# wolearyc/ramannoodle

Hardware: NVIDIA B200
Metric: md_frames_per_s (higher is better)
Workload: dtype f64

## Files before the change

ramannoodle_b200/csrc/rn_device.cuh:

```cuda
#pragma once

#include "rn_common.cuh"

namespace rn {

struct Alpha0 {
    double v[9];
};

__device__ __forceinline__ double wrap_disp(double pos, double ref) {
    const double d = pos - ref;
    return d - ceil(d - 0.5);
}

__device__ __forceinline__ double wrap_disp_fast(double pos, double ref) {
    const double d = pos - ref;
    const unsigned mag = (unsigned)__double2hiint(d) & 0x7fffffffu;
    if (mag < 0x3fe00000u) return d;
    return d - ceil(d - 0.5);
}

__device__ __forceinline__ void dmma884(double& c0, double& c1, double a, double b) {
    asm("mma.sync.aligned.m8n8k4.row.col.f64.f64.f64.f64 {%0,%1}, {%2}, {%3}, {%0,%1};"
        : "+d"(c0), "+d"(c1)
        : "d"(a), "d"(b));
}

__device__ __forceinline__ uint32_t smem_u32(const void* p) { return (uint32_t)__cvta_generic_to_shared(p); }

__device__ __forceinline__ void cp_async_16(uint32_t dst, const void* src, int src_bytes) {
    asm volatile("cp.async.cg.shared.global [%0], [%1], 16, %2;" ::"r"(dst), "l"(src), "r"(src_bytes) : "memory");
}
__device__ __forceinline__ void cp_async_8(uint32_t dst, const void* src, int src_bytes) {
    asm volatile("cp.async.ca.shared.global [%0], [%1], 8, %2;" ::"r"(dst), "l"(src), "r"(src_bytes) : "memory");
}
__device__ __forceinline__ void cp_async_commit() { asm volatile("cp.async.commit_group;" ::: "memory"); }
template <int N>
__device__ __forceinline__ void cp_async_wait() {
    asm volatile("cp.async.wait_group %0;" ::"n"(N) : "memory");
}

__device__ __forceinline__ void mbar_init(uint32_t bar, uint32_t count) {
    asm volatile("mbarrier.init.shared::cta.b64 [%0], %1;" ::"r"(bar), "r"(count) : "memory");
}
__device__ __forceinline__ void mbar_arrive_expect_tx(uint32_t bar, uint32_t bytes) {
    asm volatile("mbarrier.arrive.expect_tx.shared::cta.b64 _, [%0], %1;" ::"r"(bar), "r"(bytes) : "memory");
}
__device__ __forceinline__ void mbar_wait(uint32_t bar, uint32_t parity) {
    asm volatile(
        "{\n"
        ".reg .pred p;\n"
        "WAIT_%=:\n"
        "mbarrier.try_wait.parity.shared::cta.b64 p, [%0], %1;\n"
        "@p bra DONE_%=;\n"
        "bra WAIT_%=;\n"
        "DONE_%=:\n"
        "}\n" ::"r"(bar),
        "r"(parity)
        : "memory");
}
__device__ __forceinline__ void tma_bulk_g2s(uint32_t dst, const void* src, uint32_t bytes, uint32_t bar) {
    asm volatile("cp.async.bulk.shared::cluster.global.mbarrier::complete_tx::bytes [%0], [%1], %2, [%3];" ::"r"(dst),
                 "l"(src), "r"(bytes), "r"(bar)
                 : "memory");
}

}
```

ramannoodle_b200/csrc/rn_fft.cuh:

```cuda
#pragma once

#include "rn_common.cuh"

namespace rn {
namespace fft {

constexpr int kLog2E = 12;
constexpr int kE = 1 << kLog2E;
constexpr int kNT = 256;
constexpr int kPerThread = kE / kNT;
constexpr size_t kTileSmemBytes = (size_t)kE * sizeof(double2);

enum { OUT_PLAIN = 0, OUT_POWER = 1, OUT_PEERS = 2 };

__device__ __forceinline__ double2 cmul(double2 a, double2 b) {
    return make_double2(a.x * b.x - a.y * b.y, a.x * b.y + a.y * b.x);
}
__device__ __forceinline__ double2 cadd(double2 a, double2 b) { return make_double2(a.x + b.x, a.y + b.y); }
__device__ __forceinline__ double2 csub(double2 a, double2 b) { return make_double2(a.x - b.x, a.y - b.y); }
__device__ __forceinline__ double2 conj(double2 a) { return make_double2(a.x, -a.y); }

template <int SGN>
__device__ __forceinline__ double2 mul_i(double2 a) {
    return SGN > 0 ? make_double2(-a.y, a.x) : make_double2(a.y, -a.x);
}

template <int RADIX, int SGN>
struct Dft;

template <int SGN>
struct Dft<2, SGN> {
    static __device__ __forceinline__ void run(double2* v) {
        const double2 a = v[0];
        v[0] = cadd(a, v[1]);
        v[1] = csub(a, v[1]);
    }
};

template <int SGN>
struct Dft<4, SGN> {
    static __device__ __forceinline__ void run(double2* v) {
        const double2 s02 = cadd(v[0], v[2]), d02 = csub(v[0], v[2]);
        const double2 s13 = cadd(v[1], v[3]), d13 = mul_i<SGN>(csub(v[1], v[3]));
        v[0] = cadd(s02, s13);
        v[1] = cadd(d02, d13);
        v[2] = csub(s02, s13);
        v[3] = csub(d02, d13);
    }
};

template <int SGN>
struct Dft<8, SGN> {
    static __device__ __forceinline__ void run(double2* v) {
        double2 e[4] = {v[0], v[2], v[4], v[6]};
        double2 o[4] = {v[1], v[3], v[5], v[7]};
        Dft<4, SGN>::run(e);
        Dft<4, SGN>::run(o);
        const double h = 0.70710678118654752440;
        const double2 o1 = make_double2(h * (o[1].x - SGN * o[1].y), h * (SGN * o[1].x + o[1].y));
        const double2 o2 = mul_i<SGN>(o[2]);
        const double2 o3 = make_double2(h * (-o[3].x - SGN * o[3].y), h * (SGN * o[3].x - o[3].y));
        v[0] = cadd(e[0], o[0]);
        v[4] = csub(e[0], o[0]);
        v[1] = cadd(e[1], o1);
        v[5] = csub(e[1], o1);
        v[2] = cadd(e[2], o2);
        v[6] = csub(e[2], o2);
        v[3] = cadd(e[3], o3);
        v[7] = csub(e[3], o3);
    }
};

template <int RADIX>
struct Log2;
template <>
struct Log2<2> {
    static constexpr int value = 1;
};
template <>
struct Log2<4> {
    static constexpr int value = 2;
};
template <>
struct Log2<8> {
    static constexpr int value = 3;
};

template <int RADIX>
__device__ __forceinline__ void apply_powers(double2* x, double2 w1) {
    x[1] = cmul(x[1], w1);
    if constexpr (RADIX >= 4) {
        const double2 w2 = cmul(w1, w1);
        const double2 w3 = cmul(w2, w1);
        x[2] = cmul(x[2], w2);
        x[3] = cmul(x[3], w3);
        if constexpr (RADIX == 8) {
            const double2 w4 = cmul(w2, w2);
            x[4] = cmul(x[4], w4);
            x[5] = cmul(x[5], cmul(w4, w1));
            x[6] = cmul(x[6], cmul(w3, w3));
            x[7] = cmul(x[7], cmul(w4, w3));
        }
    }
}

template <int RADIX>
__device__ __forceinline__ void apply_base_step(double2* x, double2 base, double2 step) {
    double2 w = base;
#pragma unroll
    for (int q = 0; q < RADIX; q++) {
        x[q] = cmul(x[q], w);
        if (q + 1 < RADIX) w = cmul(w, step);
    }
}

__device__ __forceinline__ int swz(int pos) { return pos ^ ((pos >> 3) & 7); }

struct Twiddles {
    const double2* hi;
    const double2* lo;
    const double2* sub;
    int split;
};

__device__ __forceinline__ double2 tw_global(const Twiddles& T, uint32_t m) {
    return cmul(__ldg(T.hi + (m >> T.split)), __ldg(T.lo + (m & ((1u << T.split) - 1u))));
}

struct PeerOut {
    double2* ptr[8];
    int log2w;
    int log2lh;
    int rank;
    int world;
    int64_t c;
};

__host__ __device__ __forceinline__ int64_t mirror_half_slots(int log2w) { return ((int64_t)1 << (log2w - 1)) + 64; }

__device__ __forceinline__ void mirror_arcs(int o, int64_t c, int log2lh, int log2w, int64_t* near_origin,
                                            int64_t* far_top) {
    const int64_t lh = (int64_t)1 << log2lh;
    const int64_t a0 = ((int64_t)o << log2w) + (c & 1);
    *near_origin = (((c + a0) >> 1) & (lh - 1)) & ~(int64_t)31;
    *far_top = (((2 * lh + c - a0) >> 1) & (lh - 1)) | 31;
}

__device__ __forceinline__ void mirror_owner(int64_t m1, int64_t c, int log2lh, int log2w, int world, int* owner,
                                             int64_t* slot) {
    const int64_t lh = (int64_t)1 << log2lh;
    int64_t u = 2 * m1 - c;
    if (u < 0) u += 2 * lh;
    const bool far_side = u > lh;
    const int64_t a = far_side ? 2 * lh - u : u;
    const int o = min((int)(a >> log2w), world - 1);
    int64_t near_origin, far_top;
    mirror_arcs(o, c, log2lh, log2w, &near_origin, &far_top);
    *owner = o;
    *slot = far_side ? mirror_half_slots(log2w) + ((far_top - m1) & (lh - 1)) : ((m1 - near_origin) & (lh - 1));
}

struct OutSpec {
    int mode;
    double* power;
    int64_t M;
    PeerOut peers;
};

__device__ __forceinline__ void store_out(const OutSpec& out, double2* plain, int seq, int64_t m, double2 v) {
    if (out.mode == OUT_PLAIN) {
        *plain = v;
    } else if (out.mode == OUT_POWER) {
        if (m < out.M) out.power[(int64_t)seq * out.M + m] = v.x * v.x + v.y * v.y;
    } else {
        int owner;
        int64_t slot;
        mirror_owner(m, out.peers.c, out.peers.log2lh, out.peers.log2w, out.peers.world, &owner, &slot);
        const int64_t stride = 2 * mirror_half_slots(out.peers.log2w);
        out.peers.ptr[owner][(int64_t)(seq * out.peers.world + out.peers.rank) * stride + slot] = v;
    }
}

template <int SGN, int RADIX, bool LEAN, class Rd, class Wr>
__device__ __forceinline__ void fft_stage(int log2sp, int log2b, const double2* __restrict__ wsub, Rd rd, Wr wr) {
    constexpr int NB = kPerThread / RADIX;
    constexpr int LR = Log2<RADIX>::value;
    const int sp = 1 << log2sp;
    const int log2ns = log2sp - log2b + LR;
    const bool has_tw = log2sp > log2b;
#pragma unroll(LEAN ? 1 : NB)
    for (int m = 0; m < NB; m++) {
        const int u = (int)threadIdx.x + m * kNT;
        const int lo = u & (sp - 1);
        const int pos0 = ((u >> log2sp) << (log2sp + LR)) + lo;
        double2 x[RADIX];
#pragma unroll
        for (int q = 0; q < RADIX; q++) x[q] = rd(pos0 + (q << log2sp), m * RADIX + q);
        double2 w1 = make_double2(1.0, 0.0);
        if (has_tw) {
            w1 = __ldg(wsub + ((lo >> log2b) << (kLog2E - log2ns)));
            if (SGN > 0) w1.y = -w1.y;
        }
        if (SGN > 0 && has_tw) apply_powers<RADIX>(x, w1);
        Dft<RADIX, SGN>::run(x);
        if (SGN < 0 && has_tw) apply_powers<RADIX>(x, w1);
#pragma unroll
        for (int q = 0; q < RADIX; q++) wr(pos0 + (q << log2sp), m * RADIX + q, x[q]);
    }
}

struct TileParams {
    double2* X;
    int64_t seq_stride;
    int tiles_per_seq;
    const double2* H;
    double2* Hout;
    int64_t limit;
    int seq_base;
    OutSpec out;
    Twiddles tw;
};

template <bool FWD_ONLY, bool LEAN>
__global__ void __launch_bounds__(kNT, LEAN ? 3 : 2) tile_kernel(const __grid_constant__ TileParams P) {
    extern __shared__ __align__(16) unsigned char fft_smem[];
    double2* S = reinterpret_cast<double2*>(fft_smem);
    const int seq = blockIdx.x / P.tiles_per_seq;
    const int tile = blockIdx.x - seq * P.tiles_per_seq;
    const int64_t tile_base = (int64_t)tile * kE;
    double2* base = P.X + (int64_t)seq * P.seq_stride + tile_base;
    const double2* wsub = P.tw.sub;

    auto rd_s = [&](int pos, int) { return S[swz(pos)]; };
    auto wr_s = [&](int pos, int, double2 v) { S[swz(pos)] = v; };
    auto rd_g = [&](int pos, int) {
        return (tile_base + pos < P.limit) ? base[pos] : make_double2(0.0, 0.0);
    };

    fft_stage<-1, 8, LEAN>(9, 0, wsub, rd_g, wr_s);
    __syncthreads();
    fft_stage<-1, 8, LEAN>(6, 0, wsub, rd_s, wr_s);
    __syncthreads();
    fft_stage<-1, 8, LEAN>(3, 0, wsub, rd_s, wr_s);
    __syncthreads();
#pragma unroll(LEAN ? 1 : kPerThread / 8)
    for (int m = 0; m < kPerThread / 8; m++) {
        const int pos0 = ((int)threadIdx.x + m * kNT) << 3;
        double2 h[8];
        const int hu = (int)threadIdx.x + m * kNT;
        if (!FWD_ONLY) {
#pragma unroll
            for (int q = 0; q < 8; q++) h[q] = __ldg(P.H + tile_base + (q << 9) + hu);
        }
        double2 x[8];
#pragma unroll
        for (int q = 0; q < 8; q++) x[q] = S[swz(pos0 + q)];
        Dft<8, -1>::run(x);
        if (FWD_ONLY) {
#pragma unroll
            for (int q = 0; q < 8; q++) P.Hout[tile_base + (q << 9) + hu] = x[q];
        } else {
#pragma unroll
            for (int q = 0; q < 8; q++) x[q] = cmul(x[q], h[q]);
            Dft<8, +1>::run(x);
#pragma unroll
            for (int q = 0; q < 8; q++) S[swz(pos0 + q)] = x[q];
        }
    }
    if (FWD_ONLY) return;
    __syncthreads();
    fft_stage<+1, 8, LEAN>(3, 0, wsub, rd_s, wr_s);
    __syncthreads();
    fft_stage<+1, 8, LEAN>(6, 0, wsub, rd_s, wr_s);
    __syncthreads();
    auto wr_g = [&](int pos, int, double2 v) { store_out(P.out, base + pos, P.seq_base + seq, tile_base + pos, v); };
    fft_stage<+1, 8, LEAN>(9, 0, wsub, rd_s, wr_g);
}

struct LevelParams {
    double2* X;
    int64_t seq_stride;
    int log2lsub;
    int log2r;
    int nsub;
    int tw_shift;
    int64_t limit;
    int seq_base;
    OutSpec out;
    Twiddles tw;
};

__device__ __forceinline__ int rev3(int x, int groups) {
    int r = 0;
    for (int i = 0; i < groups; i++) {
        r = (r << 3) | (x & 7);
        x >>= 3;
    }
    return r;
}

template <int SGN>
struct LevelCtx {
    const LevelParams& P;
    double2* S;
    double2* base;
    int64_t elem_base;
    int seq;
    int log2b, log2s;
    int a8;
    int j0;
};

template <int SGN, int RADIX, bool SMEM_SIDE, bool LEAN>
__device__ __forceinline__ void level_twiddle_stage(const LevelCtx<SGN>& C) {
    constexpr int NB = kPerThread / RADIX;
    constexpr int LR = Log2<RADIX>::value;
    const LevelParams& P = C.P;
    const int B = 1 << C.log2b;
    const int groups = (P.log2r - LR) / 3;
#pragma unroll(LEAN ? 1 : (RADIX == 8 ? NB : 2))
    for (int m = 0; m < NB; m++) {
        const int u = (int)threadIdx.x + m * kNT;
        const int col = u & (B - 1);
        const int rb = u >> C.log2b;
        const int pos0 = (rb << (C.log2b + LR)) + col;
        const uint32_t j = (uint32_t)(C.j0 + col);
        const uint32_t krest = (uint32_t)rev3(rb, groups);
        double2 wb = tw_global(P.tw, (krest * j) << P.tw_shift);
        double2 ws = tw_global(P.tw, (j << (P.log2r - LR)) << P.tw_shift);
        if (SGN > 0) {
            wb.y = -wb.y;
            ws.y = -ws.y;
        }
        double2 x[RADIX];
        if (SGN < 0) {
#pragma unroll
            for (int q = 0; q < RADIX; q++) {
                const int pos = pos0 + (q << C.log2b);
                if (SMEM_SIDE) {
                    x[q] = C.S[swz(pos)];
                } else {
                    const int64_t off = ((int64_t)(pos >> C.log2b) << C.log2s) + (pos & (B - 1));
                    x[q] = (C.elem_base + off < P.limit) ? C.base[off] : make_double2(0.0, 0.0);
                }
            }
            Dft<RADIX, SGN>::run(x);
            apply_base_step<RADIX>(x, wb, ws);
#pragma unroll
            for (int q = 0; q < RADIX; q++) {
                const int pos = pos0 + (q << C.log2b);
                C.base[((int64_t)(pos >> C.log2b) << C.log2s) + (pos & (B - 1))] = x[q];
            }
        } else {
#pragma unroll
            for (int q = 0; q < RADIX; q++) {
                const int pos = pos0 + (q << C.log2b);
                x[q] = C.base[((int64_t)(pos >> C.log2b) << C.log2s) + (pos & (B - 1))];
            }
            apply_base_step<RADIX>(x, wb, ws);
            Dft<RADIX, SGN>::run(x);
#pragma unroll
            for (int q = 0; q < RADIX; q++) {
                const int pos = pos0 + (q << C.log2b);
                if (SMEM_SIDE) {
                    C.S[swz(pos)] = x[q];
                } else {
                    const int64_t off = ((int64_t)(pos >> C.log2b) << C.log2s) + (pos & (B - 1));
                    store_out(P.out, C.base + off, C.seq, C.elem_base + off, x[q]);
                }
            }
        }
    }
}

template <int SGN, bool LEAN>
__global__ void __launch_bounds__(kNT, LEAN ? 3 : 2) level_kernel(const __grid_constant__ LevelParams P) {
    extern __shared__ __align__(16) unsigned char fft_smem[];
    double2* S = reinterpret_cast<double2*>(fft_smem);
    const int log2b = kLog2E - P.log2r;
    const int log2s = P.log2lsub - P.log2r;
    const int log2chunks = log2s - log2b;
    const int chunk = blockIdx.x & ((1 << log2chunks) - 1);
    const int rest = blockIdx.x >> log2chunks;
    const int sub = rest % P.nsub;
    const int seq = rest / P.nsub;
    const int64_t elem_base = ((int64_t)sub << P.log2lsub) + ((int64_t)chunk << log2b);
    double2* base = P.X + (int64_t)seq * P.seq_stride + elem_base;
    const double2* wsub = P.tw.sub;
    const int a8 = P.log2r / 3, r1 = P.log2r % 3;
    const int B = 1 << log2b;
    LevelCtx<SGN> C{P, S, base, elem_base, P.seq_base + seq, log2b, log2s, a8, chunk << log2b};

    auto rd_s = [&](int pos, int) { return S[swz(pos)]; };
    auto wr_s = [&](int pos, int, double2 v) { S[swz(pos)] = v; };
    auto goff = [&](int pos) { return ((int64_t)(pos >> log2b) << log2s) + (pos & (B - 1)); };

    if (a8 + (r1 ? 1 : 0) == 1) {
        if (r1 == 1) level_twiddle_stage<SGN, 2, false, LEAN>(C);
        else if (r1 == 2) level_twiddle_stage<SGN, 4, false, LEAN>(C);
        else level_twiddle_stage<SGN, 8, false, LEAN>(C);
        return;
    }
    if constexpr (SGN < 0) {
        auto rd_g = [&](int pos, int) {
            const int64_t off = goff(pos);
            return (elem_base + off < P.limit) ? base[off] : make_double2(0.0, 0.0);
        };
        int log2sp = kLog2E - 3;
        fft_stage<-1, 8, LEAN>(log2sp, log2b, wsub, rd_g, wr_s);
        __syncthreads();
        const int mid = (r1 ? a8 : a8 - 1) - 1;
        for (int i = 0; i < mid; i++) {
            log2sp -= 3;
            fft_stage<-1, 8, LEAN>(log2sp, log2b, wsub, rd_s, wr_s);
            __syncthreads();
        }
        if (r1 == 1) level_twiddle_stage<-1, 2, true, LEAN>(C);
        else if (r1 == 2) level_twiddle_stage<-1, 4, true, LEAN>(C);
        else level_twiddle_stage<-1, 8, true, LEAN>(C);
    } else {
        if (r1 == 1) level_twiddle_stage<+1, 2, true, LEAN>(C);
        else if (r1 == 2) level_twiddle_stage<+1, 4, true, LEAN>(C);
        else level_twiddle_stage<+1, 8, true, LEAN>(C);
        __syncthreads();
        const int mid = (r1 ? a8 : a8 - 1) - 1;
        int log2sp = kLog2E - 3 * (mid + 1);
        for (int i = 0; i < mid; i++) {
            fft_stage<+1, 8, LEAN>(log2sp, log2b, wsub, rd_s, wr_s);
            __syncthreads();
            log2sp += 3;
        }
        auto wr_g = [&](int pos, int, double2 v) {
            const int64_t off = goff(pos);
            store_out(P.out, base + off, P.seq_base + seq, elem_base + off, v);
        };
        fft_stage<+1, 8, LEAN>(kLog2E - 3, log2b, wsub, rd_s, wr_g);
    }
}

}
}
```

ramannoodle_b200/csrc/rn_spectrum.cu:

```cuda
#include <algorithm>
#include <cmath>
#include <cstdlib>

#include "rn_fft.cuh"

struct rn_spectrum_plan {
    int device = 0;
    int sm_count = 0;
    int64_t S = 0, M = 0, L = 0;
    int log2l = 0;
    int world = 1;
    int rank = 0;
    int64_t Lh = 0;
    int log2lh = 0;
    int nlev = 0;
    int lev_log2r[2] = {0, 0};
    int split = 0;
    double2* d_whi = nullptr;
    double2* d_wlo = nullptr;
    double2* d_wsub = nullptr;
    double2* d_H = nullptr;
    double2* d_work = nullptr;
    double* d_power = nullptr;
    double* d_epart = nullptr;
    unsigned int* d_ticket = nullptr;
    int pack_blocks = 0;
    int64_t batch = 1;
    double* d_cross = nullptr;
    int64_t cross_doubles = 0;
};

namespace rn {

using fft::cmul;
using fft::kE;
using fft::kLog2E;
using fft::kNT;
using fft::Twiddles;

constexpr int kPackThreads = 256;
constexpr double kSqrt5 = 2.2360679774997896964;
constexpr double kSqrt5_25 = 2.2912878474779200033;
constexpr double kSqrt1_75 = 1.3228756555322952953;
constexpr double kSqrt21 = 4.5825756949558400066;

__device__ __forceinline__ double2 chirp(int64_t n, int64_t M) {
    const uint64_t m = ((uint64_t)n * (uint64_t)n) % (uint64_t)(2 * M);
    double s, c;
    sincospi((double)m / (double)M, &s, &c);
    return make_double2(c, -s);
}

static Twiddles plan_twiddles(const rn_spectrum_plan* p) {
    Twiddles t;
    t.hi = p->d_whi;
    t.lo = p->d_wlo;
    t.sub = p->d_wsub;
    t.split = p->split;
    return t;
}

struct PackParams {
    const double* src;
    int64_t M;
    int64_t Lh;
    int64_t begin, end;
    double2* dst[8];
    int aligned16;
    int seq_sel;
    double* epart;
    unsigned int* ticket;
    double* share[8];
    int num_share;
    int share_slot;
    int zero_slot;
    int log2_stripe;
    int phase;
    Twiddles tw;
    int64_t win_stride;
};

__device__ __forceinline__ double block_sum(double v, double* sm) {
    const int lane = threadIdx.x & 31, warp = threadIdx.x >> 5;
#pragma unroll
    for (int off = 16; off > 0; off >>= 1) v += __shfl_xor_sync(0xffffffffu, v, off);
    if (lane == 0) sm[warp] = v;
    __syncthreads();
    double total = 0.0;
    if (threadIdx.x == 0)
        for (int w = 0; w < (int)(blockDim.x >> 5); w++) total += sm[w];
    return total;
}

__device__ __forceinline__ void publish_energy(double block_total, double* epart, unsigned int* ticket, double* red,
                                               const PackParams* share = nullptr) {
    __shared__ bool last;
    if (threadIdx.x == 0) {
        epart[blockIdx.x] = block_total;
        __threadfence();
        last = atomicAdd(ticket, 1u) == gridDim.x - 1;
    }
    __syncthreads();
    if (!last) return;
    __threadfence();
    double v = 0.0;
    for (unsigned int b = threadIdx.x; b < gridDim.x; b += blockDim.x) v += __ldcg(epart + b);
    __syncthreads();
    const double total = block_sum(v, red);
    if (threadIdx.x == 0) {
        epart[gridDim.x] = total;
        *ticket = 0;
        if (share)
            for (int d = 0; d < share->num_share; d++) {
                share->share[d][share->share_slot] = total;
                if (share->zero_slot >= 0) share->share[d][share->zero_slot] = 0.0;
            }
    }
}

template <int G, bool WIN = false>
__global__ void __launch_bounds__(kPackThreads) pack_alpha_kernel(const __grid_constant__ PackParams P) {
    static_assert(!WIN || G == 1, "windows are packed for single-GPU transforms only");
    constexpr int GH = G > 1 ? G / 2 : 1;
    __shared__ __align__(16) double rows[(kPackThreads + 1) * 9 + 1];
    __shared__ double red[kPackThreads / 32];
    const double* src = P.src;
    double2* dst0 = P.dst[0];
    double* epart = P.epart;
    unsigned int* ticket = P.ticket;
    bool aligned16 = P.aligned16;
    if constexpr (WIN) {
        src += (int64_t)blockIdx.y * P.win_stride;
        dst0 += (int64_t)blockIdx.y * 3 * P.Lh;
        epart += (int64_t)blockIdx.y * (gridDim.x + 1);
        ticket += blockIdx.y;
        aligned16 = reinterpret_cast<uintptr_t>(src) % 16 == 0;
    }
    int64_t n0 = P.begin + (int64_t)blockIdx.x * kPackThreads;
    if (P.log2_stripe >= 0) {
        const int64_t idx = (int64_t)blockIdx.x * kPackThreads, stripe = (int64_t)1 << P.log2_stripe;
        n0 = P.begin + ((idx >> P.log2_stripe) << (P.log2_stripe + 1)) + (idx & (stripe - 1)) + P.phase * stripe;
    }
    const int64_t n1 = n0 + threadIdx.x;
    double2 a[GH][3];
    double energy = 0.0;
#pragma unroll
    for (int q = 0; q < GH; q++) {
        const int64_t first = (int64_t)q * P.Lh + n0;
        const int64_t avail = min((int64_t)kPackThreads + 1, P.M + 1 - first);
        __syncthreads();
        const int64_t valid = avail > 0 ? avail * 9 : 0;
        if (aligned16) {
            constexpr int kVec = ((kPackThreads + 1) * 9 + 1) / 2;
            constexpr int kPer = (kVec + kPackThreads - 1) / kPackThreads;
            const double2* src2 = reinterpret_cast<const double2*>(src + first * 9);
            double2 staged[kPer];
#pragma unroll
            for (int i = 0; i < kPer; i++) {
                const int e = threadIdx.x + i * kPackThreads;
                staged[i] = make_double2(0.0, 0.0);
                if (2 * e + 1 < valid) staged[i] = __ldg(src2 + e);
                else if (2 * e < valid) staged[i].x = __ldg(src + first * 9 + 2 * e);
            }
#pragma unroll
            for (int i = 0; i < kPer; i++) {
                const int e = threadIdx.x + i * kPackThreads;
                if (e < kVec) {
                    rows[2 * e] = staged[i].x;
                    if (2 * e + 1 < (kPackThreads + 1) * 9) rows[2 * e + 1] = staged[i].y;
                }
            }
        } else {
            for (int e = threadIdx.x; e < (kPackThreads + 1) * 9; e += kPackThreads)
                rows[e] = (e < valid) ? __ldg(src + first * 9 + e) : 0.0;
        }
        __syncthreads();
        const int64_t n = first + threadIdx.x;
#pragma unroll
        for (int s = 0; s < 3; s++) a[q][s] = make_double2(0.0, 0.0);
        if (n < P.M && n1 < P.end) {
            const double* r = rows + threadIdx.x * 9;
            const double xx = r[9] - r[0], yy = r[13] - r[4], zz = r[17] - r[8];
// ... 236 lines not shown
        wn_out[k] = wavenumber_of(k, M, dt);
    }
}


constexpr int kCrossTile = 4;

__device__ __forceinline__ int64_t upper_pair(int64_t g, int64_t h, int64_t G) {
    return g * (2 * G - g - 1) / 2 + (h - g - 1);
}

__device__ __forceinline__ void md_signals(const double* __restrict__ r0, double z[6]) {
    const double* r1 = r0 + 9;
    const double xx = __ldg(r1 + 0) - __ldg(r0 + 0), yy = __ldg(r1 + 4) - __ldg(r0 + 4);
    const double zz = __ldg(r1 + 8) - __ldg(r0 + 8), xy = __ldg(r1 + 1) - __ldg(r0 + 1);
    const double yz = __ldg(r1 + 5) - __ldg(r0 + 5), xz = __ldg(r1 + 2) - __ldg(r0 + 2);
    z[0] = kSqrt5 * (xx + yy + zz);
    z[1] = kSqrt5_25 * (xx - zz);
    z[2] = kSqrt1_75 * (xx - 2.0 * yy + zz);
    z[3] = kSqrt21 * xy;
    z[4] = kSqrt21 * yz;
    z[5] = kSqrt21 * xz;
}

__global__ void __launch_bounds__(256) cross_energy_kernel(const double* __restrict__ src, int64_t stride, int G,
                                                           int64_t M, double* __restrict__ part,
                                                           double* __restrict__ energy, unsigned int* ticket) {
    __shared__ double red[kCrossTile][8];
    __shared__ bool last;
    const int lane = threadIdx.x & 31, warp = threadIdx.x >> 5;
    const int64_t n = (int64_t)blockIdx.x * blockDim.x + threadIdx.x;
    for (int g0 = 0; g0 < G - 1; g0 += kCrossTile) {
        double zg[kCrossTile][6];
#pragma unroll
        for (int r = 0; r < kCrossTile; r++) {
#pragma unroll
            for (int i = 0; i < 6; i++) zg[r][i] = 0.0;
            if (n < M && g0 + r < G) md_signals(src + (int64_t)(g0 + r) * stride + n * 9, zg[r]);
        }
        for (int h = g0 + 1; h < G; h++) {
            double zh[6] = {0.0, 0.0, 0.0, 0.0, 0.0, 0.0};
            if (n < M) md_signals(src + (int64_t)h * stride + n * 9, zh);
#pragma unroll
            for (int r = 0; r < kCrossTile; r++) {
                double v = (zg[r][0] * zh[0] + zg[r][1] * zh[1]) + (zg[r][2] * zh[2] + zg[r][3] * zh[3]) +
                           (zg[r][4] * zh[4] + zg[r][5] * zh[5]);
#pragma unroll
                for (int off = 16; off > 0; off >>= 1) v += __shfl_xor_sync(0xffffffffu, v, off);
                if (lane == 0) red[r][warp] = v;
            }
            __syncthreads();
            if (threadIdx.x < kCrossTile && g0 + (int)threadIdx.x < h) {
                const int r = threadIdx.x;
                double total = 0.0;
                for (int w = 0; w < (int)(blockDim.x >> 5); w++) total += red[r][w];
                part[upper_pair(g0 + r, h, G) * gridDim.x + blockIdx.x] = total;
                __threadfence();
            }
            __syncthreads();
        }
    }
    if (threadIdx.x == 0) last = atomicAdd(ticket, 1u) == gridDim.x - 1;
    __syncthreads();
    if (!last) return;
    __threadfence();
    const int64_t pairs = (int64_t)G * (G - 1) / 2;
    for (int64_t p = warp; p < pairs; p += blockDim.x >> 5) {
        double v = 0.0;
        for (unsigned int b = lane; b < gridDim.x; b += 32) v += __ldcg(part + p * gridDim.x + b);
#pragma unroll
        for (int off = 16; off > 0; off >>= 1) v += __shfl_xor_sync(0xffffffffu, v, off);
        if (lane == 0) energy[p] = v;
    }
    if (threadIdx.x == 0) *ticket = 0;
}

__device__ __forceinline__ double re_dot(double2 a, double2 b) { return a.x * b.x + a.y * b.y; }

__global__ void __launch_bounds__(256) cross_combine_kernel(const double2* __restrict__ y, int64_t Lh, int G,
                                                            const double* __restrict__ epart, int64_t epart_stride,
                                                            const double* __restrict__ energy, int64_t M,
                                                            double scale, int64_t points, SpectrumParams prm,
                                                            double* __restrict__ wn_out, double* __restrict__ int_out) {
    for (int64_t g = blockIdx.y; g < G; g += gridDim.y) {
        const double2* yg = y + 3 * g * Lh;
        for (int64_t o = blockIdx.x * (int64_t)blockDim.x + threadIdx.x; o < points;
             o += (int64_t)gridDim.x * blockDim.x) {
            const int64_t k = o + 1;
            double2 a[3][2];
#pragma unroll
            for (int s = 0; s < 3; s++) {
                a[s][0] = yg[s * Lh + k];
                a[s][1] = yg[s * Lh + (M - k)];
            }
            const double wn = wavenumber_of(k, M, prm.timestep);
            if (g == 0) wn_out[o] = wn;
            for (int64_t h = g; h < G; h++) {
                const double2* yh = y + 3 * h * Lh;
                double sum = 0.0;
#pragma unroll
                for (int s = 0; s < 3; s++)
                    sum = __dadd_rn(sum, __dadd_rn(re_dot(a[s][0], yh[s * Lh + k]), re_dot(a[s][1], yh[s * Lh + (M - k)])));
                const double e = h == g ? epart[g * epart_stride] : energy[upper_pair(g, h, G)];
                const double econst = 0.5 * e;
                const double inten = corrected(sum * scale + econst, wn, prm);
                int_out[(g * G + h) * points + o] = inten;
                if (h != g) int_out[(h * G + g) * points + o] = inten;
            }
        }
    }
}

static int grid_for(int64_t n, int sms) {
    return (int)std::max<int64_t>(1, std::min<int64_t>((n + 255) / 256, (int64_t)sms * 16));
}

static int ensure_smem_attr(int device) {
    static std::atomic<bool> done[64];
    if (device >= 0 && device < 64 && done[device].load(std::memory_order_acquire)) return RN_OK;
#define RN_FFT_SMEM(kern) \
    RN_CUDA(cudaFuncSetAttribute(kern, cudaFuncAttributeMaxDynamicSharedMemorySize, (int)fft::kTileSmemBytes))
    RN_FFT_SMEM((fft::tile_kernel<false, false>));
    RN_FFT_SMEM((fft::tile_kernel<false, true>));
    RN_FFT_SMEM((fft::tile_kernel<true, false>));
    RN_FFT_SMEM((fft::level_kernel<-1, false>));
    RN_FFT_SMEM((fft::level_kernel<-1, true>));
    RN_FFT_SMEM((fft::level_kernel<+1, false>));
    RN_FFT_SMEM((fft::level_kernel<+1, true>));
#undef RN_FFT_SMEM
    if (device >= 0 && device < 64) done[device].store(true, std::memory_order_release);
    return RN_OK;
}

static int fft_lean() {
    static const int value = [] {
        const char* env = getenv("RN_FFT_LEAN");
        return env ? atoi(env) : 3;
    }();
    return value;
}

static fft::OutSpec plain_out() {
    fft::OutSpec o;
    o.mode = fft::OUT_PLAIN;
    o.power = nullptr;
    o.M = 0;
    for (int i = 0; i < 8; i++) o.peers.ptr[i] = nullptr;
    o.peers.log2w = 0;
    o.peers.rank = 0;
    o.peers.world = 1;
    return o;
}

template <int SGN>
static int launch_level(const rn_spectrum_plan* p, double2* X, int nseq, int seq_base, int lev, int64_t limit,
                        const fft::OutSpec& out, cudaStream_t stream) {
    fft::LevelParams P;
    P.X = X;
    P.seq_base = seq_base;
    P.seq_stride = p->Lh;
    int log2lsub = p->log2lh;
    for (int i = 0; i < lev; i++) log2lsub -= p->lev_log2r[i];
    P.log2lsub = log2lsub;
    P.log2r = p->lev_log2r[lev];
    P.nsub = (int)(p->Lh >> log2lsub);
    P.tw_shift = p->log2l - log2lsub;
    P.limit = limit;
    P.out = out;
    P.tw = plan_twiddles(p);
    const int64_t grid = (int64_t)nseq * (p->Lh >> kLog2E);
    if (fft_lean() & 1) fft::level_kernel<SGN, true><<<(unsigned)grid, kNT, fft::kTileSmemBytes, stream>>>(P);
    else fft::level_kernel<SGN, false><<<(unsigned)grid, kNT, fft::kTileSmemBytes, stream>>>(P);
    RN_LAUNCHED();
    RN_CUDA(cudaGetLastError());
    return RN_OK;
}

static int run_convolution(const rn_spectrum_plan* p, double2* X, int nseq, int64_t limit, const fft::OutSpec& out,
                           double2* hout, cudaStream_t stream, int seq_base = 0) {
    int rc = ensure_smem_attr(p->device);
    if (rc != RN_OK) return rc;
    const fft::OutSpec plain = plain_out();
    for (int lev = 0; lev < p->nlev; lev++) {
        rc = launch_level<-1>(p, X, nseq, seq_base, lev, lev == 0 ? limit : p->Lh, plain, stream);
        if (rc != RN_OK) return rc;
    }
    fft::TileParams T;
    T.X = X;
    T.seq_stride = p->Lh;
    T.tiles_per_seq = (int)(p->Lh >> kLog2E);
    T.H = p->d_H;
    T.Hout = hout;
    T.limit = p->nlev == 0 ? limit : p->Lh;
    T.seq_base = seq_base;
    T.out = p->nlev == 0 ? out : plain;
    T.tw = plan_twiddles(p);
    const unsigned grid = (unsigned)((int64_t)nseq * T.tiles_per_seq);
    if (hout) fft::tile_kernel<true, false><<<grid, kNT, fft::kTileSmemBytes, stream>>>(T);
    else if (fft_lean() & 2) fft::tile_kernel<false, true><<<grid, kNT, fft::kTileSmemBytes, stream>>>(T);
    else fft::tile_kernel<false, false><<<grid, kNT, fft::kTileSmemBytes, stream>>>(T);
    RN_LAUNCHED();
    RN_CUDA(cudaGetLastError());
    if (hout) return RN_OK;
    for (int lev = p->nlev - 1; lev >= 0; lev--) {
        rc = launch_level<+1>(p, X, nseq, seq_base, lev, p->Lh, lev == 0 ? out : plain, stream);
        if (rc != RN_OK) return rc;
    }
    return RN_OK;
}

static void destroy_plan(rn_spectrum_plan* p) {
    if (!p) return;
    cudaFree(p->d_whi);
    cudaFree(p->d_wlo);
    cudaFree(p->d_wsub);
    cudaFree(p->d_H);
    cudaFree(p->d_work);
    cudaFree(p->d_power);
    cudaFree(p->d_epart);
    cudaFree(p->d_ticket);
    cudaFree(p->d_cross);
    delete p;
}

static double2 unit_root(int64_t num, int64_t den) {
    const long double two_pi = 6.283185307179586476925286766559005768L;
    const long double ang = two_pi * (long double)num / (long double)den;
    return make_double2((double)cosl(ang), (double)-sinl(ang));
}

constexpr int64_t kMaxBatch = 65535;

static int create_plan(int64_t num_frames, int device, int world, int rank, rn_spectrum_plan** out,
                       int64_t batch = 1) {
    RN_CHECK_ARG(out != nullptr, "out is null");
    *out = nullptr;
    RN_CHECK_ARG(num_frames >= 2, "a spectrum needs at least 2 frames (got %lld)", (long long)num_frames);
    RN_CHECK_ARG(world >= 1 && world <= 8 && rank >= 0 && rank < world, "invalid rank %d of %d", rank, world);
    RN_CHECK_ARG(batch >= 1 && batch <= kMaxBatch && (batch == 1 || world == 1),
                 "invalid batch %lld (1 .. %lld windows, single-GPU plans only)", (long long)batch,
                 (long long)kMaxBatch);
    int count = 0;
    RN_CUDA(cudaGetDeviceCount(&count));
    RN_CHECK_ARG(device >= 0 && device < count, "device %d out of range (%d devices)", device, count);
    DeviceGuard guard(device);
    if (!guard.ok) {
        set_error("cudaSetDevice(%d) failed", device);
        return RN_ERR_CUDA;
    }
    cudaDeviceProp prop;
    RN_CUDA(cudaGetDeviceProperties(&prop, device));
    int group = 1;
    while (group * 2 <= world) group *= 2;
    const int64_t M = num_frames - 1;
    int log2l = kLog2E;
    while (((int64_t)1 << log2l) < std::max<int64_t>(2 * M - 1, (int64_t)kE * group)) log2l++;
    RN_CHECK_ARG(log2l <= 30, "series too long for one spectrum plan (%lld frames)", (long long)num_frames);
    RN_CHECK_ARG(3 * batch * (((int64_t)1 << log2l) >> kLog2E) <= (int64_t)INT32_MAX,
                 "batch %lld too large for windows of %lld frames", (long long)batch, (long long)num_frames);
    rn_spectrum_plan* p = new rn_spectrum_plan();
    p->batch = batch;
    p->device = device;
    p->sm_count = prop.multiProcessorCount;
    p->S = num_frames;
    p->M = M;
    p->log2l = log2l;
    p->L = (int64_t)1 << log2l;
    p->world = group;
    p->rank = rank;
    p->Lh = p->L / group;
    p->log2lh = log2l;
    for (int g = group; g > 1; g >>= 1) p->log2lh--;
    const int q = p->log2lh - kLog2E;
    if (q == 0) {
        p->nlev = 0;
    } else if (q <= 10) {
        p->nlev = 1;
        p->lev_log2r[0] = q;
    } else {
        p->nlev = 2;
        p->lev_log2r[0] = (q + 1) / 2;
        p->lev_log2r[1] = q - p->lev_log2r[0];
    }
    const int64_t owned = rank < group ? (group > 1 ? p->Lh / group : M) : 0;
    p->pack_blocks = (int)((owned + kPackThreads - 1) / kPackThreads);
    if (rank >= group) {
        *out = p;
        return RN_OK;
    }
    p->split = log2l / 2;
    const int64_t n_hi = p->L >> p->split, n_lo = (int64_t)1 << p->split;
    cudaError_t err = cudaSuccess;
    auto alloc = [&](void** ptr, size_t bytes) {
        if (err == cudaSuccess) err = cudaMalloc(ptr, bytes);
    };
    alloc((void**)&p->d_whi, sizeof(double2) * n_hi);
    alloc((void**)&p->d_wlo, sizeof(double2) * n_lo);
    alloc((void**)&p->d_wsub, sizeof(double2) * kE);
    alloc((void**)&p->d_H, sizeof(double2) * p->Lh);
    const int64_t psets = std::max<int64_t>(2, batch);
    alloc((void**)&p->d_work, sizeof(double2) * (group > 1 ? 1 : 3 * batch) * p->Lh);
    if (group == 1) alloc((void**)&p->d_power, sizeof(double) * 3 * batch * M);
    alloc((void**)&p->d_epart, sizeof(double) * psets * (p->pack_blocks + 1));
    alloc((void**)&p->d_ticket, psets * sizeof(unsigned int));
    if (err != cudaSuccess) {
        set_error("cudaMalloc failed while creating a spectrum plan for %lld frames: %s", (long long)num_frames,
                  cudaGetErrorString(err));
        destroy_plan(p);
        cudaGetLastError();
        return RN_ERR_OUT_OF_MEMORY;
    }
    cudaMemset(p->d_ticket, 0, psets * sizeof(unsigned int));
    std::vector<double2> whi((size_t)n_hi), wlo((size_t)n_lo), wsub((size_t)kE);
    for (int64_t a = 0; a < n_hi; a++) whi[(size_t)a] = unit_root(a << p->split, p->L);
    for (int64_t b = 0; b < n_lo; b++) wlo[(size_t)b] = unit_root(b, p->L);
    for (int m = 0; m < kE; m++) wsub[(size_t)m] = unit_root(m, kE);
    cudaError_t e1 = cudaMemcpy(p->d_whi, whi.data(), sizeof(double2) * n_hi, cudaMemcpyHostToDevice);
    if (e1 == cudaSuccess) e1 = cudaMemcpy(p->d_wlo, wlo.data(), sizeof(double2) * n_lo, cudaMemcpyHostToDevice);
    if (e1 == cudaSuccess) e1 = cudaMemcpy(p->d_wsub, wsub.data(), sizeof(double2) * kE, cudaMemcpyHostToDevice);
    if (e1 != cudaSuccess) {
        set_error("twiddle table upload failed: %s", cudaGetErrorString(e1));
        destroy_plan(p);
        return RN_ERR_CUDA;
    }
    filter_fill_kernel<<<grid_for(p->Lh, p->sm_count), 256>>>(p->d_work, M, p->L, p->Lh, group, rank, plan_twiddles(p));
    RN_LAUNCHED();
    int rc = run_convolution(p, p->d_work, 1, p->Lh, plain_out(), p->d_H, nullptr);
    if (rc == RN_OK) {
        cudaError_t e2 = cudaStreamSynchronize(nullptr);
        if (e2 != cudaSuccess) {
            set_error("spectrum plan initialisation failed: %s", cudaGetErrorString(e2));
            rc = RN_ERR_CUDA;
        }
    }
    if (rc != RN_OK) {
        destroy_plan(p);
        return rc;
    }
    if (group > 1) {
        cudaFree(p->d_work);
        p->d_work = nullptr;
    }
    *out = p;
    return RN_OK;
}

static SpectrumParams spectrum_params(double timestep_fs, int laser, double laser_wavelength_nm, int be,
                                      double temperature_K) {
    SpectrumParams prm;
    prm.timestep = timestep_fs;
    prm.laser = laser ? 1 : 0;
    prm.laser_wavenumber = laser ? 10000000.0 / laser_wavelength_nm : 0.0;
    prm.bose_einstein = be ? 1 : 0;
    prm.kt = 8.617333262e-5 * temperature_K;
    return prm;
}

static PackParams md_pack_params(const rn_spectrum_plan* plan, const double* d_alpha) {
    PackParams pp;
    pp.src = d_alpha;
    pp.M = plan->M;
    pp.Lh = plan->Lh;
    pp.begin = 0;
    pp.end = plan->M;
    for (int i = 0; i < 8; i++) pp.dst[i] = nullptr;
    pp.dst[0] = plan->d_work;
    pp.aligned16 = (reinterpret_cast<uintptr_t>(pp.src) % 16 == 0) ? 1 : 0;
    pp.seq_sel = -1;
    pp.num_share = 0;
    pp.share_slot = 0;
    pp.zero_slot = -1;
    pp.log2_stripe = -1;
    pp.phase = 0;
    for (int i = 0; i < 8; i++) pp.share[i] = nullptr;
    pp.epart = plan->d_epart;
    pp.ticket = plan->d_ticket;
    pp.tw = plan_twiddles(plan);
    pp.win_stride = 0;
    return pp;
}

}

using namespace rn;

extern "C" int64_t rn_spectrum_num_points(int64_t num_frames) {
    const int64_t M = num_frames - 1;
    if (M < 1) return 0;
    return (M + 1) / 2 - 1;
}

extern "C" int rn_spectrum_plan_create(int64_t num_frames, int device, rn_spectrum_plan** out) {
    return create_plan(num_frames, device, 1, 0, out);
}

extern "C" int rn_spectrum_plan_create_batched(int64_t window_frames, int64_t batch, int device,
                                               rn_spectrum_plan** out) {
    return create_plan(window_frames, device, 1, 0, out, batch);
}

extern "C" int rn_spectrum_plan_create_dist(int64_t num_frames, int device, int world, int rank,
                                            rn_spectrum_plan** out) {
    return create_plan(num_frames, device, world, rank, out);
}

extern "C" int rn_spectrum_plan_destroy(rn_spectrum_plan* plan) {
    if (!plan) return RN_OK;
    DeviceGuard guard(plan->device);
    destroy_plan(plan);
    return RN_OK;
}

extern "C" int rn_spectrum_plan_info(const rn_spectrum_plan* plan, int64_t info[8]) {
    RN_CHECK_ARG(plan != nullptr && info != nullptr, "null pointer");
    info[0] = plan->log2l;
    info[1] = plan->world;
    info[2] = plan->log2lh;
    info[3] = plan->nlev;
    info[4] = plan->lev_log2r[0];
    info[5] = plan->lev_log2r[1];
    info[6] = plan->world > 1 ? plan->Lh / plan->world : plan->Lh;
    info[7] = plan->M;
    return RN_OK;
}

extern "C" int rn_md_spectrum(rn_spectrum_plan* plan, const double* d_alpha, double timestep_fs, int laser_correction,
                              double laser_wavelength_nm, int bose_einstein_correction, double temperature_K,
                              double* d_wavenumbers, double* d_intensities, void* stream) {
    RN_CHECK_ARG(plan != nullptr, "plan is null");
    RN_CHECK_ARG(plan->world == 1, "rn_md_spectrum needs a single-GPU plan (rn_spectrum_plan_create)");
    RN_CHECK_ARG(d_alpha != nullptr, "d_alpha is null");
    RN_CHECK_ARG(timestep_fs > 0, "timestep must be positive");
    if (laser_correction) RN_CHECK_ARG(laser_wavelength_nm > 0, "invalid laser_wavelength");
    if (bose_einstein_correction) RN_CHECK_ARG(temperature_K > 0, "invalid temperature: %g <= 0", temperature_K);
    const int64_t points = rn_spectrum_num_points(plan->S);
    if (points == 0) return RN_OK;
    RN_CHECK_ARG(d_wavenumbers && d_intensities, "null output pointer");
    DeviceGuard guard(plan->device);
    cudaStream_t s = static_cast<cudaStream_t>(stream);
    const int64_t M = plan->M;

    const PackParams pp = md_pack_params(plan, d_alpha);
    pack_alpha_kernel<1><<<plan->pack_blocks, kPackThreads, 0, s>>>(pp);
    RN_LAUNCHED();
    fft::OutSpec out = plain_out();
    out.mode = fft::OUT_POWER;
    out.power = plan->d_power;
    out.M = M;
    int rc = run_convolution(plan, plan->d_work, 3, M, out, nullptr, s);
    if (rc != RN_OK) return rc;
    const SpectrumParams prm = spectrum_params(timestep_fs, laser_correction, laser_wavelength_nm,
                                               bose_einstein_correction, temperature_K);
    const double scale = 0.25 / ((double)plan->L * (double)plan->L);
    combine_md_kernel<<<grid_for(points, plan->sm_count), 256, 0, s>>>(plan->d_power, 3, plan->d_epart + plan->pack_blocks, 1,
                                                                      M, scale, points, prm, d_wavenumbers, d_intensities);
    RN_LAUNCHED();
    RN_CUDA(cudaGetLastError());
    return RN_OK;
}

extern "C" int rn_md_spectrum_windows(rn_spectrum_plan* plan, const double* d_alpha, int64_t num_frames,
                                      int64_t hop_frames, double timestep_fs, int laser_correction,
                                      double laser_wavelength_nm, int bose_einstein_correction, double temperature_K,
                                      double* d_wavenumbers, double* d_intensities, void* stream) {
    RN_CHECK_ARG(plan != nullptr, "plan is null");
    RN_CHECK_ARG(plan->world == 1, "rn_md_spectrum_windows needs a single-GPU plan (rn_spectrum_plan_create_batched)");
    RN_CHECK_ARG(d_alpha != nullptr, "d_alpha is null");
    RN_CHECK_ARG(num_frames >= plan->S, "a window of %lld frames does not fit a series of %lld frames",
                 (long long)plan->S, (long long)num_frames);
    RN_CHECK_ARG(hop_frames >= 1, "hop_frames must be at least 1 (got %lld)", (long long)hop_frames);
    RN_CHECK_ARG(timestep_fs > 0, "timestep must be positive");
    if (laser_correction) RN_CHECK_ARG(laser_wavelength_nm > 0, "invalid laser_wavelength");
    if (bose_einstein_correction) RN_CHECK_ARG(temperature_K > 0, "invalid temperature: %g <= 0", temperature_K);
    const int64_t points = rn_spectrum_num_points(plan->S);
    if (points == 0) return RN_OK;
    RN_CHECK_ARG(d_wavenumbers && d_intensities, "null output pointer");
    DeviceGuard guard(plan->device);
    cudaStream_t s = static_cast<cudaStream_t>(stream);
    const int64_t M = plan->M;
    const int64_t windows = 1 + (num_frames - plan->S) / hop_frames;
    const SpectrumParams prm = spectrum_params(timestep_fs, laser_correction, laser_wavelength_nm,
                                               bose_einstein_correction, temperature_K);
    const double scale = 0.25 / ((double)plan->L * (double)plan->L);
    for (int64_t first = 0; first < windows; first += plan->batch) {
        const int64_t nb = std::min(plan->batch, windows - first);
        PackParams pp = md_pack_params(plan, d_alpha + first * hop_frames * 9);
        pp.win_stride = hop_frames * 9;
        pack_alpha_kernel<1, true><<<dim3(plan->pack_blocks, (unsigned)nb), kPackThreads, 0, s>>>(pp);
        RN_LAUNCHED();
        fft::OutSpec out = plain_out();
        out.mode = fft::OUT_POWER;
        out.power = plan->d_power;
        out.M = M;
        int rc = run_convolution(plan, plan->d_work, (int)(3 * nb), M, out, nullptr, s);
// ... 314 lines not shown
```

Before: 1.010 billion.

## Load forward FFT input tiles via TMA tensor maps instead of per-thread reads

Replaces the first-stage per-thread global loads in the tile and forward level kernels with a 5D TMA tensor copy into 1024-aligned shared memory, completed on an mbarrier. Out-of-range elements are handled by TMA bounds plus an explicit zeroing pass for the straddling row. Tensor maps are encoded on the host through the driver entry point and cached per plan. The aim is to cut load-issue overhead and improve coalescing. In exchange it adds host-side encoding, a mutex-guarded cache, and a serialized wait before compute starts.

```diff
diff --git a/ramannoodle_b200/csrc/rn_device.cuh b/ramannoodle_b200/csrc/rn_device.cuh
--- a/ramannoodle_b200/csrc/rn_device.cuh
+++ b/ramannoodle_b200/csrc/rn_device.cuh
@@ -64,5 +64,13 @@
                  "l"(src), "r"(bytes), "r"(bar)
                  : "memory");
 }
+__device__ __forceinline__ void tma_tensor_g2s_5d(uint32_t dst, const void* map, int c0, int c1, int c2, int c3, int c4,
+                                                  uint32_t bar) {
+    asm volatile(
+        "cp.async.bulk.tensor.5d.shared::cluster.global.tile.mbarrier::complete_tx::bytes [%0], [%1, {%2, %3, %4, %5, "
+        "%6}], [%7];" ::"r"(dst),
+        "l"(reinterpret_cast<uint64_t>(map)), "r"(c0), "r"(c1), "r"(c2), "r"(c3), "r"(c4), "r"(bar)
+        : "memory");
+}
 
 }
diff --git a/ramannoodle_b200/csrc/rn_fft.cuh b/ramannoodle_b200/csrc/rn_fft.cuh
--- a/ramannoodle_b200/csrc/rn_fft.cuh
+++ b/ramannoodle_b200/csrc/rn_fft.cuh
@@ -1,6 +1,9 @@
 #pragma once
 
+#include <cuda.h>
+
 #include "rn_common.cuh"
+#include "rn_device.cuh"
 
 namespace rn {
 namespace fft {
@@ -9,7 +12,8 @@
 constexpr int kE = 1 << kLog2E;
 constexpr int kNT = 256;
 constexpr int kPerThread = kE / kNT;
-constexpr size_t kTileSmemBytes = (size_t)kE * sizeof(double2);
+constexpr uint32_t kTileBytes = (uint32_t)(kE * sizeof(double2));
+constexpr size_t kTileSmemBytes = (size_t)kTileBytes + sizeof(uint64_t);
 
 enum { OUT_PLAIN = 0, OUT_POWER = 1, OUT_PEERS = 2 };
 
@@ -116,6 +120,37 @@
 
 __device__ __forceinline__ int swz(int pos) { return pos ^ ((pos >> 3) & 7); }
 
+__device__ __forceinline__ double2* tile_smem(unsigned char* raw) {
+    if (smem_u32(raw) & 1023u) __trap();
+    return reinterpret_cast<double2*>(raw);
+}
+__device__ __forceinline__ uint64_t* tile_bar(double2* S) { return reinterpret_cast<uint64_t*>(S + kE); }
+
+__device__ __forceinline__ void land_tile(const CUtensorMap* map, double2* S, uint64_t* bar, int log2r, int piece,
+                                          int sub, int seq) {
+    const uint32_t b = smem_u32(bar);
+    if (threadIdx.x == 0) {
+        mbar_init(b, 1);
+        asm volatile("fence.proxy.async.shared::cta;" ::: "memory");
+        mbar_arrive_expect_tx(b, kTileBytes);
+        const int box_rows = min(1 << log2r, 256);
+        for (int r = 0; r < (1 << log2r); r += box_rows)
+            tma_tensor_g2s_5d(smem_u32(S + (r << (kLog2E - log2r))), map, 0, piece, r, sub, seq, b);
+    }
+    __syncthreads();
+    mbar_wait(b, 0);
+}
+
+__device__ __forceinline__ void zero_straddle(double2* S, int64_t rel, int log2r, int log2b, int log2s, int j0) {
+    const int64_t r0 = rel >> log2s;
+    const int jl = (int)(rel & ((1 << log2s) - 1));
+    const int c0 = max(jl - j0, 0);
+    if (r0 >= (1 << log2r) || jl == 0 || c0 >= (1 << log2b)) return;
+    for (int c = c0 + (int)threadIdx.x; c < (1 << log2b); c += kNT)
+        S[swz(((int)r0 << log2b) + c)] = make_double2(0.0, 0.0);
+    __syncthreads();
+}
+
 struct Twiddles {
     const double2* hi;
     const double2* lo;
@@ -219,12 +254,13 @@
     int seq_base;
     OutSpec out;
     Twiddles tw;
+    CUtensorMap map;
 };
 
 template <bool FWD_ONLY, bool LEAN>
 __global__ void __launch_bounds__(kNT, LEAN ? 3 : 2) tile_kernel(const __grid_constant__ TileParams P) {
-    extern __shared__ __align__(16) unsigned char fft_smem[];
-    double2* S = reinterpret_cast<double2*>(fft_smem);
+    extern __shared__ __align__(1024) unsigned char fft_smem[];
+    double2* S = tile_smem(fft_smem);
     const int seq = blockIdx.x / P.tiles_per_seq;
     const int tile = blockIdx.x - seq * P.tiles_per_seq;
     const int64_t tile_base = (int64_t)tile * kE;
@@ -233,11 +269,10 @@
 
     auto rd_s = [&](int pos, int) { return S[swz(pos)]; };
     auto wr_s = [&](int pos, int, double2 v) { S[swz(pos)] = v; };
-    auto rd_g = [&](int pos, int) {
-        return (tile_base + pos < P.limit) ? base[pos] : make_double2(0.0, 0.0);
-    };
-
-    fft_stage<-1, 8, LEAN>(9, 0, wsub, rd_g, wr_s);
+
+    land_tile(&P.map, S, tile_bar(S), 9, 0, tile, seq);
+    zero_straddle(S, P.limit - tile_base, 9, 3, 3, 0);
+    fft_stage<-1, 8, LEAN>(9, 0, wsub, rd_s, wr_s);
     __syncthreads();
     fft_stage<-1, 8, LEAN>(6, 0, wsub, rd_s, wr_s);
     __syncthreads();
@@ -288,6 +323,7 @@
     int seq_base;
     OutSpec out;
     Twiddles tw;
+    CUtensorMap map;
 };
 
 __device__ __forceinline__ int rev3(int x, int groups) {
@@ -375,8 +411,8 @@
 
 template <int SGN, bool LEAN>
 __global__ void __launch_bounds__(kNT, LEAN ? 3 : 2) level_kernel(const __grid_constant__ LevelParams P) {
-    extern __shared__ __align__(16) unsigned char fft_smem[];
-    double2* S = reinterpret_cast<double2*>(fft_smem);
+    extern __shared__ __align__(1024) unsigned char fft_smem[];
+    double2* S = tile_smem(fft_smem);
     const int log2b = kLog2E - P.log2r;
     const int log2s = P.log2lsub - P.log2r;
     const int log2chunks = log2s - log2b;
@@ -402,12 +438,18 @@
         return;
     }
     if constexpr (SGN < 0) {
-        auto rd_g = [&](int pos, int) {
-            const int64_t off = goff(pos);
-            return (elem_base + off < P.limit) ? base[off] : make_double2(0.0, 0.0);
-        };
         int log2sp = kLog2E - 3;
-        fft_stage<-1, 8, LEAN>(log2sp, log2b, wsub, rd_g, wr_s);
+        if (log2b >= 3) {
+            land_tile(&P.map, S, tile_bar(S), P.log2r, chunk << (log2b - 3), sub, seq);
+            zero_straddle(S, P.limit - ((int64_t)sub << P.log2lsub), P.log2r, log2b, log2s, chunk << log2b);
+            fft_stage<-1, 8, LEAN>(log2sp, log2b, wsub, rd_s, wr_s);
+        } else {
+            auto rd_g = [&](int pos, int) {
+                const int64_t off = goff(pos);
+                return (elem_base + off < P.limit) ? base[off] : make_double2(0.0, 0.0);
+            };
+            fft_stage<-1, 8, LEAN>(log2sp, log2b, wsub, rd_g, wr_s);
+        }
         __syncthreads();
         const int mid = (r1 ? a8 : a8 - 1) - 1;
         for (int i = 0; i < mid; i++) {
diff --git a/ramannoodle_b200/csrc/rn_spectrum.cu b/ramannoodle_b200/csrc/rn_spectrum.cu
--- a/ramannoodle_b200/csrc/rn_spectrum.cu
+++ b/ramannoodle_b200/csrc/rn_spectrum.cu
@@ -1,8 +1,20 @@
+#include <cudaTypedefs.h>
+
 #include <algorithm>
 #include <cmath>
 #include <cstdlib>
+#include <mutex>
 
 #include "rn_fft.cuh"
+
+struct rn_fft_maps {
+    const void* X = nullptr;
+    int64_t nseq = 0;
+    int64_t limit = 0;
+    CUtensorMap first{};
+    CUtensorMap level1{};
+    CUtensorMap tile{};
+};
 
 struct rn_spectrum_plan {
     int device = 0;
@@ -28,6 +40,8 @@
     int64_t batch = 1;
     double* d_cross = nullptr;
     int64_t cross_doubles = 0;
+    std::vector<rn_fft_maps> maps;
+    std::mutex maps_mutex;
 };
 
 namespace rn {
@@ -570,15 +584,95 @@
     return o;
 }
 
+static PFN_cuTensorMapEncodeTiled_v12000 tensor_map_encoder() {
+    static const PFN_cuTensorMapEncodeTiled_v12000 fn = [] {
+        void* f = nullptr;
+        cudaDriverEntryPointQueryResult q = cudaDriverEntryPointSymbolNotFound;
+        if (cudaGetDriverEntryPoint("cuTensorMapEncodeTiled", &f, cudaEnableDefault, &q) != cudaSuccess ||
+            q != cudaDriverEntryPointSuccess) {
+            cudaGetLastError();
+            f = nullptr;
+        }
+        return reinterpret_cast<PFN_cuTensorMapEncodeTiled_v12000>(f);
+    }();
+    return fn;
+}
+
+static int encode_tile_map(CUtensorMap* map, const void* X, int64_t nseq, int64_t Lh, int log2lsub, int log2r,
+                           int64_t limit) {
+    const PFN_cuTensorMapEncodeTiled_v12000 encode = tensor_map_encoder();
+    if (!encode) {
+        set_error("cuTensorMapEncodeTiled is not available from the CUDA driver");
+        return RN_ERR_CUDA;
+    }
+    const int log2b = kLog2E - log2r, log2s = log2lsub - log2r;
+    const int64_t R = (int64_t)1 << log2r, s = (int64_t)1 << log2s, lsub = (int64_t)1 << log2lsub;
+    RN_CHECK_ARG(log2b >= 3 && limit >= 1 && (limit >= lsub || lsub == Lh), "invalid tile map geometry");
+    const int64_t rows = limit >= lsub ? R : std::min(R, (limit + s - 1) >> log2s);
+    const cuuint64_t dims[5] = {16, (cuuint64_t)(s >> 3), (cuuint64_t)rows, (cuuint64_t)(Lh >> log2lsub),
+                                (cuuint64_t)nseq};
+    const cuuint64_t strides[4] = {128, (cuuint64_t)(s * 16), (cuuint64_t)(lsub * 16), (cuuint64_t)(Lh * 16)};
+    const cuuint32_t box[5] = {16, (cuuint32_t)(1 << (log2b - 3)), (cuuint32_t)std::min<int64_t>(R, 256), 1, 1};
+    const cuuint32_t estride[5] = {1, 1, 1, 1, 1};
+    const CUresult r = encode(map, CU_TENSOR_MAP_DATA_TYPE_FLOAT64, 5, const_cast<void*>(X), dims, strides, box,
+                              estride, CU_TENSOR_MAP_INTERLEAVE_NONE, CU_TENSOR_MAP_SWIZZLE_128B,
+                              CU_TENSOR_MAP_L2_PROMOTION_L2_256B, CU_TENSOR_MAP_FLOAT_OOB_FILL_NONE);
+    if (r != CUDA_SUCCESS) {
+        set_error("cuTensorMapEncodeTiled failed (%d) for a tile map of 2^%d rows", (int)r, log2r);
+        return RN_ERR_CUDA;
+    }
+    return RN_OK;
+}
+
+static int log2lsub_of(const rn_spectrum_plan* p, int lev) {
+    int log2lsub = p->log2lh;
+    for (int i = 0; i < lev; i++) log2lsub -= p->lev_log2r[i];
+    return log2lsub;
+}
+
+static bool level_uses_map(const rn_spectrum_plan* p, int lev) {
+    return p->lev_log2r[lev] >= 4 && p->lev_log2r[lev] <= kLog2E - 3;
+}
+
+static int encode_fft_maps(const rn_spectrum_plan* p, rn_fft_maps* m) {
+    const int64_t nseq = m->nseq;
+    if (p->nlev == 0) return encode_tile_map(&m->first, m->X, nseq, p->Lh, kLog2E, 9, m->limit);
+    int rc = encode_tile_map(&m->tile, m->X, nseq, p->Lh, kLog2E, 9, p->Lh);
+    if (rc == RN_OK && level_uses_map(p, 0))
+        rc = encode_tile_map(&m->first, m->X, nseq, p->Lh, p->log2lh, p->lev_log2r[0], m->limit);
+    if (rc == RN_OK && p->nlev == 2 && level_uses_map(p, 1))
+        rc = encode_tile_map(&m->level1, m->X, nseq, p->Lh, log2lsub_of(p, 1), p->lev_log2r[1], p->Lh);
+    return rc;
+}
+
+static int fft_maps(rn_spectrum_plan* p, const void* X, int64_t nseq, int64_t limit, rn_fft_maps* out) {
+    if (X == p->d_work) nseq = 3 * p->batch;
+    std::lock_guard<std::mutex> lock(p->maps_mutex);
+    for (const rn_fft_maps& m : p->maps)
+        if (m.X == X && m.nseq == nseq && m.limit == limit) {
+            *out = m;
+            return RN_OK;
+        }
+    rn_fft_maps m;
+    m.X = X;
+    m.nseq = nseq;
+    m.limit = limit;
+    const int rc = encode_fft_maps(p, &m);
+    if (rc != RN_OK) return rc;
+    if (p->maps.size() >= 32) p->maps.clear();
+    p->maps.push_back(m);
+    *out = m;
+    return RN_OK;
+}
+
 template <int SGN>
 static int launch_level(const rn_spectrum_plan* p, double2* X, int nseq, int seq_base, int lev, int64_t limit,
-                        const fft::OutSpec& out, cudaStream_t stream) {
-    fft::LevelParams P;
+                        const CUtensorMap* map, const fft::OutSpec& out, cudaStream_t stream) {
+    fft::LevelParams P{};
     P.X = X;
     P.seq_base = seq_base;
     P.seq_stride = p->Lh;
-    int log2lsub = p->log2lh;
-    for (int i = 0; i < lev; i++) log2lsub -= p->lev_log2r[i];
+    const int log2lsub = log2lsub_of(p, lev);
     P.log2lsub = log2lsub;
     P.log2r = p->lev_log2r[lev];
     P.nsub = (int)(p->Lh >> log2lsub);
@@ -586,6 +680,7 @@
     P.limit = limit;
     P.out = out;
     P.tw = plan_twiddles(p);
+    if (map) P.map = *map;
     const int64_t grid = (int64_t)nseq * (p->Lh >> kLog2E);
     if (fft_lean() & 1) fft::level_kernel<SGN, true><<<(unsigned)grid, kNT, fft::kTileSmemBytes, stream>>>(P);
     else fft::level_kernel<SGN, false><<<(unsigned)grid, kNT, fft::kTileSmemBytes, stream>>>(P);
@@ -594,13 +689,17 @@
     return RN_OK;
 }
 
-static int run_convolution(const rn_spectrum_plan* p, double2* X, int nseq, int64_t limit, const fft::OutSpec& out,
+static int run_convolution(rn_spectrum_plan* p, double2* X, int nseq, int64_t limit, const fft::OutSpec& out,
                            double2* hout, cudaStream_t stream, int seq_base = 0) {
     int rc = ensure_smem_attr(p->device);
     if (rc != RN_OK) return rc;
+    rn_fft_maps maps;
+    rc = fft_maps(p, X, nseq, limit, &maps);
+    if (rc != RN_OK) return rc;
     const fft::OutSpec plain = plain_out();
     for (int lev = 0; lev < p->nlev; lev++) {
-        rc = launch_level<-1>(p, X, nseq, seq_base, lev, lev == 0 ? limit : p->Lh, plain, stream);
+        rc = launch_level<-1>(p, X, nseq, seq_base, lev, lev == 0 ? limit : p->Lh, lev == 0 ? &maps.first : &maps.level1,
+                              plain, stream);
         if (rc != RN_OK) return rc;
     }
     fft::TileParams T;
@@ -613,6 +712,7 @@
     T.seq_base = seq_base;
     T.out = p->nlev == 0 ? out : plain;
     T.tw = plan_twiddles(p);
+    T.map = p->nlev == 0 ? maps.first : maps.tile;
     const unsigned grid = (unsigned)((int64_t)nseq * T.tiles_per_seq);
     if (hout) fft::tile_kernel<true, false><<<grid, kNT, fft::kTileSmemBytes, stream>>>(T);
     else if (fft_lean() & 2) fft::tile_kernel<false, true><<<grid, kNT, fft::kTileSmemBytes, stream>>>(T);
@@ -621,7 +721,7 @@
     RN_CUDA(cudaGetLastError());
     if (hout) return RN_OK;
     for (int lev = p->nlev - 1; lev >= 0; lev--) {
-        rc = launch_level<+1>(p, X, nseq, seq_base, lev, p->Lh, lev == 0 ? out : plain, stream);
+        rc = launch_level<+1>(p, X, nseq, seq_base, lev, p->Lh, nullptr, lev == 0 ? out : plain, stream);
         if (rc != RN_OK) return rc;
     }
     return RN_OK;
@@ -744,6 +844,10 @@
     filter_fill_kernel<<<grid_for(p->Lh, p->sm_count), 256>>>(p->d_work, M, p->L, p->Lh, group, rank, plan_twiddles(p));
     RN_LAUNCHED();
     int rc = run_convolution(p, p->d_work, 1, p->Lh, plain_out(), p->d_H, nullptr);
+    if (rc == RN_OK && group == 1) {
+        rn_fft_maps maps;
+        rc = fft_maps(p, p->d_work, 1, M, &maps);
+    }
     if (rc == RN_OK) {
         cudaError_t e2 = cudaStreamSynchronize(nullptr);
         if (e2 != cudaSuccess) {
@@ -758,6 +862,7 @@
     if (group > 1) {
         cudaFree(p->d_work);
         p->d_work = nullptr;
+        p->maps.clear();
     }
     *out = p;
     return RN_OK;
```

Result: no change. 1.013 billion (median of 6 runs) (+0.3%).
